# morrislab/rnascan

Measured on AMD Instinct MI355X. Metric: scored windows/sec (seq+struct, w=12), higher is better.
Workload: dtype f64

## Files before the change

### include/pfmscan.h

```cpp
#ifndef PFMSCAN_H
#define PFMSCAN_H

#include <stdint.h>

#ifdef __cplusplus
extern "C" {
#endif

#define PFMSCAN_ABI_VERSION 27
#define PFMSCAN_NCODE   8
#define PFMSCAN_SEP     7
#define PFMSCAN_NSTRUCT 7
#define PFMSCAN_MAX_M   64
#define PFMSCAN_MAX_WIDTH 4096
#define PFMSCAN_SITE_GROUP 4096
#define PFMSCAN_SITE_LIMBS 66
#define PFMSCAN_SITE_JOINT_COLS 64

#define PFMSCAN_OK          0
#define PFMSCAN_E_BADARG   -1
#define PFMSCAN_E_BADSHAPE -2
#define PFMSCAN_E_OOM      -3
#define PFMSCAN_E_HIP      -4
#define PFMSCAN_E_CAPACITY -5
// ... 151 lines not shown
int pfmscan_debug_pair_credits(const double *letters_seq, const double *letters_struct, int m, double thr_sum,
                               uint16_t *credits_seq, uint16_t *credits_struct, double *quantum, double *slack,
                               double *thr_joint, double *survive, int *mode);
int pfmscan_debug_pair_sum_test(const float *seq, const double *st, int64_t n, double thr_sum,
                                uint8_t *maybe, uint8_t *passes, double *margin0);

typedef struct pfmscan_library pfmscan_library;
int pfmscan_library_create(pfmscan_ctx *ctx, const double *letter_tables,
                           const double *struct_pssms, int n_motifs, int m,
                           pfmscan_library **out);
void pfmscan_library_destroy(pfmscan_library *lib);
int pfmscan_library_info(const pfmscan_library *lib, int *n_motifs, int *m, int *n_passes,
                         int *motifs_per_pass, double *max_eps);
int pfmscan_library_last_launches(const pfmscan_library *lib, int *n_launches, int *n_team_launches,
                                  int *max_teams);
int pfmscan_library_hits_dev(pfmscan_ctx *ctx, pfmscan_library *lib,
                             const uint8_t *d_codes, const void *d_profile,
                             int profile_dtype, int64_t n_pos, const double *thr_seq,
                             const double *thr_struct, int64_t capacity,
                             int64_t *d_hit_pos, int32_t *d_hit_motif, float *d_hit_seq,
                             double *d_hit_struct, uint64_t *d_hit_count, void *stream);
int pfmscan_library_hits_staged(pfmscan_ctx *ctx, pfmscan_library *lib,
                                const double *thr_seq, const double *thr_struct,
                                int64_t capacity, int64_t *hit_pos, int32_t *hit_motif,
                                float *hit_seq, double *hit_struct, int64_t *n_hits);
int pfmscan_library_hits_host(pfmscan_ctx *ctx, pfmscan_library *lib,
                              const uint8_t *codes, const void *profile, int profile_dtype,
                              int64_t n_pos, const double *thr_seq, const double *thr_struct,
                              int64_t capacity, int64_t *hit_pos, int32_t *hit_motif,
                              float *hit_seq, double *hit_struct, int64_t *n_hits);
// ... 48 lines not shown
                                         int64_t *d_hit_pos, int32_t *d_hit_motif, float *d_hit_seq,
                                         double *d_hit_struct, uint64_t *d_hit_count, void *stream);
int pfmscan_library_hits_letters_sum_host(pfmscan_ctx *ctx, pfmscan_library *lib, const uint8_t *codes,
                                          const uint8_t *codes2, int64_t n_pos, const double *thr_seq,
                                          const double *thr_struct, const double *thr_sum, int64_t capacity,
                                          int64_t *hit_pos, int32_t *hit_motif, float *hit_seq,
                                          double *hit_struct, int64_t *n_hits);
int pfmscan_library_letters_sum_thresholds(const double *letter_tables, const double *struct_tables, int n_motifs,
                                           int m, const double *thr_seq, const double *thr_sum, double *thr_eff);

int pfmscan_debug_credit_table(const double *letter_table, int m, double thr_seq, int bits,
                               uint16_t *credits, double *slack);

int pfmscan_debug_library8_credits(const double *letter_table, int m, double thr, uint16_t *credits, double *slack);

int pfmscan_debug_credit8_table(const double *letter_table, int m, double thr, uint16_t *credits, int *mode);

#define PFMSCAN_UPLOAD_RUNTIME 0
#define PFMSCAN_UPLOAD_STAGED  1
int pfmscan_set_upload_mode(pfmscan_ctx *ctx, int mode);
int pfmscan_upload_source_file(pfmscan_ctx *ctx, const void *base, size_t length, const char *path, int64_t file_offset);
int pfmscan_upload_source_file_checked(pfmscan_ctx *ctx, const void *base, size_t length, const char *path,
                                       int64_t file_offset, int64_t st_dev, int64_t st_ino, int64_t st_size);

int pfmscan_dotbracket_annotate_dev(pfmscan_ctx *ctx, const uint8_t *d_in, uint8_t *d_out, int64_t n_pos,
                                    const uint8_t *map, int64_t *d_counts, int64_t *first_bad, void *stream);
int pfmscan_dotbracket_stage(pfmscan_ctx *ctx, const uint8_t *codes, int64_t n_pos, int which, const uint8_t *map,
                             int64_t *counts, int64_t *first_bad);
int pfmscan_dotbracket_annotate_host(pfmscan_ctx *ctx, const uint8_t *in, uint8_t *out, int64_t n_pos,
                                     const uint8_t *map, int64_t *counts, int64_t *first_bad);
// ... 297 lines not shown
```

### rnascan_amd/_lib.py

```python
import ctypes
import importlib.util
import os
import sys

import numpy as np

HERE = os.path.dirname(os.path.abspath(__file__))
LIB_PATH = os.environ.get("PFMSCAN_LIB") or os.path.join(HERE, "libpfmscan.so")

OK = 0
E_BADARG, E_BADSHAPE, E_OOM, E_HIP, E_CAPACITY = -1, -2, -3, -4, -5
PROFILE_NONE, PROFILE_F32, PROFILE_F64 = 0, 1, 2
SEP = 7
NCODE = 8
NSTRUCT = 7
MAX_M = 64
MAX_WIDTH = 4096
ABI_VERSION = 27

SYMBOLS = [
    "pfmscan_abi_version", "pfmscan_ctx_create", "pfmscan_ctx_destroy", "pfmscan_last_error",
    "pfmscan_device_info", "pfmscan_synchronize", "pfmscan_motif_create", "pfmscan_motif_destroy",
    "pfmscan_pwm_calculate", "pfmscan_scan_dev", "pfmscan_scan_letters_f64_dev", "pfmscan_hits_dev",
    "pfmscan_scan_host", "pfmscan_scan_letters_f64_host", "pfmscan_hits_host", "pfmscan_time_scan_dev",
# ... 23 lines not shown
    "pfmscan_site_joint_dev", "pfmscan_site_joint_staged",
    "pfmscan_mutmap_dev", "pfmscan_mutmap_staged", "pfmscan_mutmap_events_dev", "pfmscan_mutmap_events_staged",
    "pfmscan_variants_dev", "pfmscan_variants_staged",
    "pfmscan_occupancy_dev", "pfmscan_occupancy_staged",
    "pfmscan_occupancy_profile_dev", "pfmscan_occupancy_profile_staged",
    "pfmscan_expect_dev", "pfmscan_expect_staged",
    "pfmscan_expect_profile_dev", "pfmscan_expect_profile_staged",
    "pfmscan_occupancy_pair_dev", "pfmscan_occupancy_pair_staged", "pfmscan_expect_pair_dev", "pfmscan_expect_pair_staged",
    "pfmscan_expect_merge_dev", "pfmscan_expect_merged_staged", "pfmscan_expect_profile_merged_staged", "pfmscan_expect_pair_merged_staged",
    "pfmscan_expect_pair_joint_dev", "pfmscan_expect_pair_joint_staged", "pfmscan_expect_pair_joint_merged_staged",
    "pfmscan_expect_profile_joint_dev", "pfmscan_expect_profile_joint_staged", "pfmscan_expect_profile_joint_merged_staged",
    "pfmscan_footprint_dev", "pfmscan_footprint_staged", "pfmscan_footprint_events_dev", "pfmscan_footprint_events_staged",
    "pfmscan_footprint_profile_dev", "pfmscan_footprint_profile_staged", "pfmscan_footprint_profile_events_dev", "pfmscan_footprint_profile_events_staged",
    "pfmscan_mutocc_dev", "pfmscan_mutocc_staged", "pfmscan_mutocc_events_dev", "pfmscan_mutocc_events_staged",
    "pfmscan_multisite_dev", "pfmscan_multisite_staged", "pfmscan_multisite_events_dev", "pfmscan_multisite_events_staged",
]
PAIR_ROUTE_NONE, PAIR_ROUTE_FUSED, PAIR_ROUTE_TWO_PHASE, PAIR_ROUTE_DENSE, PAIR_ROUTE_CREDITS = range(5)
SITE_GROUP = 4096
SITE_LIMBS = 66
SITE_JOINT_COLS = 64
EXPECT_RATIO, EXPECT_POSTERIOR = 0, 1
OCC_FANIN = 32
FOOTPRINT_SLOTS = 512
FOOTPRINT_PROFILE_SLOTS = 256
MULTISITE_SLOTS = 512
MULTISITE_CHUNK = 28
MUTOCC_TILE = 512
MAX_COVER = 1024
AVG_OK, AVG_DOTBRACKET, AVG_UNCOVERED, AVG_COVER, AVG_BAD_TABLE = range(5)
TSV_CONST, TSV_I64, TSV_F32, TSV_F64, TSV_INDEXED, TSV_FIXED, TSV_WINDOW, TSV_SPAN = range(8)

# ... 2045 lines not shown
                                                                 dtype=np.float64), (self.n,)))
        return ts, tt

    def info(self):
        n, m, npass, per, eps = ctypes.c_int(), ctypes.c_int(), ctypes.c_int(), ctypes.c_int(), ctypes.c_double()
        self._ctx._check(self._L.pfmscan_library_info(self._h, ctypes.byref(n), ctypes.byref(m), ctypes.byref(npass),
                                                      ctypes.byref(per), ctypes.byref(eps)))
        return {"n_motifs": n.value, "m": m.value, "passes": npass.value, "motifs_per_pass": per.value,
                "max_prefilter_eps": eps.value}

    def last_launches(self):
        n, teams, most = ctypes.c_int(), ctypes.c_int(), ctypes.c_int()
        self._ctx._check(self._L.pfmscan_library_last_launches(self._h, ctypes.byref(n), ctypes.byref(teams), ctypes.byref(most)))
        return {"n_launches": n.value, "n_team_launches": teams.value, "max_teams": most.value}

    def close(self):
        if getattr(self, "_h", None) and getattr(self._ctx, "_h", None):
            self._L.pfmscan_library_destroy(self._h)
        self._h = None

    def __del__(self):
        try:
            self.close()
        except Exception:
            pass


def credit_table(letter_table, thr_seq, bits=16):
    L = load()
    T = np.ascontiguousarray(letter_table, dtype=np.float64)
# ... 25 lines not shown


def library8_credits(letter_table, thr):
    L = load()
    T = np.ascontiguousarray(letter_table, dtype=np.float64)
    if T.ndim != 2 or T.shape[1] != NCODE:
        raise ValueError("letter_table must be [m][8]")
    rows = (T.shape[0] + 3) // 4 * 4
    out = np.zeros((rows, 8), dtype=np.uint16)
    slack = ctypes.c_double(0.0)
    L.pfmscan_debug_library8_credits.argtypes = [ctypes.c_void_p, ctypes.c_int, ctypes.c_double, ctypes.c_void_p, ctypes.POINTER(ctypes.c_double)]
    rc = L.pfmscan_debug_library8_credits(_ptr(T), T.shape[0], float(thr), _ptr(out), ctypes.byref(slack))
    if rc != OK:
        raise ValueError("pfmscan_debug_library8_credits: bad argument")
    return out, slack.value


def credit8_table(letter_table, thr):
    L = load()
    T = np.ascontiguousarray(letter_table, dtype=np.float64)
    if T.ndim != 2 or T.shape[1] != NCODE:
        raise ValueError("letter_table must be [m][8]")
    out = np.zeros((T.shape[0], 8), dtype=np.uint16)
    mode = ctypes.c_int(0)
    rc = L.pfmscan_debug_credit8_table(_ptr(T), T.shape[0], float(thr), _ptr(out), ctypes.byref(mode))
    if rc != OK:
        raise ValueError("pfmscan_debug_credit8_table: bad argument")
    return out, mode.value


# ... 26 lines not shown
```

### rnascan_amd/build.py

```python
import os
import re
import shutil
import subprocess
import sys
import tempfile
from concurrent.futures import ThreadPoolExecutor

HERE = os.path.dirname(os.path.abspath(__file__))
CSRC = os.path.join(HERE, "csrc")
OBJ = os.path.join(CSRC, "_obj")
LIB = os.path.join(HERE, "libpfmscan.so")
SOURCES = ["pfmscan_kernels.hip", "pfmscan_letters8.hip", "pfmscan_pairsum.hip", "pfmscan_letters_fixed.hip", "pfmscan_api.hip", "pfmscan_hits.hip", "pfmscan_sort.hip", "pfmscan_library.hip", "pfmscan_library_api.hip", "pfmscan_proflib.hip", "pfmscan_profile_fixed.hip", "pfmscan_place.hip",
           "pfmscan_pipeline.hip", "pfmscan_ingest.hip", "pfmscan_upload.hip", "pfmscan_dotbracket.hip", "pfmscan_average.hip", "pfmscan_background.hip", "pfmscan_rowbound.hip", "pfmscan_sites.hip", "pfmscan_sites_host.hip", "pfmscan_sites_lib.hip",
           "pfmscan_sites_lib_host.hip", "pfmscan_sites_letters.hip", "pfmscan_mutation.hip", "pfmscan_occupancy.hip", "pfmscan_expect.hip", "pfmscan_expect_profile.hip", "pfmscan_expect_merge.hip", "pfmscan_footprint.hip", "pfmscan_footprint_profile.hip", "pfmscan_mutocc.hip", "pfmscan_multisite.hip"]
HEADERS = ["pfmscan_internal.hpp", "pfmscan_ctx.hpp", "pfmscan_hits.hpp", "pfmscan_hitqueue.hpp", "pfmscan_device.hpp", "pfmscan_profile.hpp", "pfmscan_exact.hpp", "pfmscan_sites.hpp", "pfmscan_superacc.hpp", "pfmscan_occ.hpp", "pfmscan_occ_plan.hpp", "pfmscan_fp.hpp", "pfmscan_fp_plan.hpp", "pfmscan_ms_plan.hpp", os.path.join("..", "..", "include", "pfmscan.h")]
DEPS = SOURCES + HEADERS
FLAGS = ["-O3", "--offload-arch=gfx950", "-std=c++17", "-fPIC", "-fno-fast-math", "-Wall"]


def hipcc_path():
    for cand in (os.environ.get("HIPCC"), shutil.which("hipcc"), "/opt/rocm/bin/hipcc"):
        if cand and os.path.exists(cand):
            return cand
    raise RuntimeError("hipcc not found (set HIPCC or install ROCm under /opt/rocm)")


def stale():
    if not os.path.exists(LIB):
        return True
    t = os.path.getmtime(LIB)
# ... 78 lines not shown
```

### rnascan_amd/csrc/pfmscan_internal.hpp

```cpp
#pragma once
#include <hip/hip_runtime.h>
#include <stdint.h>
#include <atomic>
#include "../../include/pfmscan.h"

namespace pfmscan {

struct CredCache {
    double thr = __builtin_nan("");
    int mode = 0;
    uint16_t cr[16 * 16];
};

struct Cred8Cache {
    double thr = __builtin_nan("");
    int mode = 0;
    uint16_t cr[32 * 8];
};

struct PairCred {
    int mode = 0;
    int m = 0;
    double thr_sum = __builtin_nan("");
    double thr_joint = 0.0, quantum = 0.0, slack = 0.0, survive = 0.0;
// ... 166 lines not shown
    const double *thr;
    double struct_band;
    const int32_t *finite;
    int n_motifs, m, motif_base;
    int64_t pos_offset;
    int64_t capacity;
    int hit_shards;
    int64_t *hit_pos;
    int32_t *hit_motif;
    double *hit_struct;
    unsigned long long *hit_count;
};
hipError_t launch_profile_library(const ProfLibArgs &a, hipStream_t stream);
int64_t profile_library_tile();

hipError_t sort_temp_bytes(int64_t total, int key_bits, size_t *bytes);
hipError_t launch_gather_sorted(const GatherArgs &g, hipStream_t stream);

}
```

### rnascan_amd/csrc/pfmscan_library_api.hip

```cpp
#include <algorithm>
#include <cmath>
#include <cstdlib>
#include <cstring>
#include <new>
#include <string>
#include <vector>

#include "pfmscan_hits.hpp"

using namespace pfmscan;

namespace {

struct LibPass {
    int motif_base = 0, n_real = 0, nmp = 0, ng = 0;
    int ng_real = 0;
    size_t pairs_off = 0;
    size_t letters_off = 0;
    size_t pssm_off = 0;
    size_t thr_off = 0;
};

}

// ... 69 lines not shown
    bool all_finite = false;
    double struct_band = 0.0;
    std::vector<double> pairsum;
    std::vector<LibPass> passes;
    uint16_t *d_pairs = nullptr;
    double *d_letters = nullptr, *d_pssm = nullptr, *d_thr = nullptr;
    size_t pairs_elems = 0, thr_elems = 0;
    std::vector<uint16_t> h_pairs;
    std::vector<double> h_thr;
    std::vector<double> cur_seq, cur_struct, eps;
    std::vector<double> h_letters, h_pssm;
    std::vector<double> band;
    std::vector<double> cur_eff, cur_sum;
    bool thr_valid = false;
    int last_launches = 0, last_team_launches = 0, last_max_teams = 0;
};

static int lib_fail(pfmscan_ctx *ctx, int code, const std::string &msg) { return fail(ctx, code, msg); }

extern "C" {

static int create_seq_library(pfmscan_ctx *ctx, const double *letter_tables, const double *struct_pssms, int ncol, int n_motifs, int m,
                              pfmscan_library **out);

int pfmscan_library_create(pfmscan_ctx *ctx, const double *letter_tables, const double *struct_pssms, int n_motifs, int m,
                           pfmscan_library **out)
{
    if (!ctx || !out || (!letter_tables && !struct_pssms)) return lib_fail(ctx, PFMSCAN_E_BADARG, "pfmscan_library_create: NULL argument");
    *out = nullptr;
    if (n_motifs < 1 || n_motifs > 65535) return lib_fail(ctx, PFMSCAN_E_BADSHAPE, "library size outside 1..65535");
// ... 2 lines not shown
    if (!letter_tables) {
        HIP_TRY(ctx, hipSetDevice(ctx->device));
        pfmscan_library *lib = new (std::nothrow) pfmscan_library();
        if (!lib) return lib_fail(ctx, PFMSCAN_E_OOM, "out of host memory");
        lib->ctx = ctx;
        lib->n = n_motifs;
        lib->m = m;
        lib->has_struct = true;
        lib->has_letters = false;
        for (int k = 0; k < n_motifs; ++k) lib->struct_band = std::max(lib->struct_band, struct_band(struct_pssms + (size_t)k * m * 7, m));
        std::vector<int32_t> fin((size_t)n_motifs, 1);
        for (int k = 0; k < n_motifs; ++k)
            for (int i = 0; i < m * 7; ++i)
                if (!std::isfinite(struct_pssms[(size_t)k * m * 7 + i])) fin[(size_t)k] = 0;
        if (std::getenv("PFMSCAN_FORCE_GENERIC")) std::fill(fin.begin(), fin.end(), 0);
        const size_t cells = (size_t)n_motifs * m * 7;
        hipError_t e = hipMalloc((void **)&lib->d_pssm_rows, cells * 8);
        if (e == hipSuccess) e = hipMemcpy(lib->d_pssm_rows, struct_pssms, cells * 8, hipMemcpyHostToDevice);
        if (e == hipSuccess) e = hipMalloc((void **)&lib->d_finite, (size_t)n_motifs * 4);
        if (e == hipSuccess) e = hipMemcpy(lib->d_finite, fin.data(), (size_t)n_motifs * 4, hipMemcpyHostToDevice);
        if (e == hipSuccess) e = hipMalloc((void **)&lib->d_thr, (size_t)n_motifs * 8);
        lib->thr_elems = (size_t)n_motifs;
        if (e != hipSuccess) {
            pfmscan_library_destroy(lib);
            return fail_hip(ctx, e, "uploading the library tables");
        }
        *out = lib;
        return PFMSCAN_OK;
    }
    return create_seq_library(ctx, letter_tables, struct_pssms, 7, n_motifs, m, out);
}

}

static int create_seq_library(pfmscan_ctx *ctx, const double *letter_tables, const double *struct_pssms, int ncol, int n_motifs, int m,
                              pfmscan_library **out)
{
// ... 171 lines not shown
            return lib_fail(ctx, PFMSCAN_E_BADSHAPE, "column 7 of every letter table must be NaN (the foreign code)");
    if (seq_tables) return create_seq_library(ctx, seq_tables, struct_tables, 8, n_motifs, m, out);
    return create_letters8_library(ctx, struct_tables, n_motifs, m, out);
}

void pfmscan_library_destroy(pfmscan_library *lib)
{
    if (!lib) return;
    if (lib->ctx) (void)hipSetDevice(lib->ctx->device);
    if (lib->d_pairs) (void)hipFree(lib->d_pairs);
    if (lib->d_letters) (void)hipFree(lib->d_letters);
    if (lib->d_pssm) (void)hipFree(lib->d_pssm);
    if (lib->d_thr) (void)hipFree(lib->d_thr);
    if (lib->d_pssm_rows) (void)hipFree(lib->d_pssm_rows);
    if (lib->d_finite) (void)hipFree(lib->d_finite);
    delete lib;
}

int pfmscan_debug_credit_table(const double *letter_table, int m, double thr_seq, int bits, uint16_t *credits, double *slack)
{
    if (!letter_table || !credits || m < 1 || m > PFMSCAN_MAX_M || std::isnan(thr_seq)) return PFMSCAN_E_BADARG;
    if (bits == 0) bits = lib_credit_bits(lib_np_bucket(m));
    if (bits != 10 && bits != 16) return PFMSCAN_E_BADARG;
    const int npair = (m + 1) / 2;
    std::vector<double> ps((size_t)npair * 16);
    pair_sums(letter_table, m, ps.data());
    const double s = build_credits(ps.data(), npair, thr_seq, credits, bits);
    if (slack) *slack = s;
    return PFMSCAN_OK;
}
// ... 23 lines not shown
        for (double v : lib->eps) mx = std::max(mx, v);
        *max_eps = lib->thr_valid ? mx : NAN;
    }
    return PFMSCAN_OK;
}

int pfmscan_library_last_launches(const pfmscan_library *lib, int *n_launches, int *n_team_launches, int *max_teams)
{
    if (!lib) return PFMSCAN_E_BADARG;
    if (n_launches) *n_launches = lib->last_launches;
    if (n_team_launches) *n_team_launches = lib->last_team_launches;
    if (max_teams) *max_teams = lib->last_max_teams;
    return PFMSCAN_OK;
}

}

static int lib_set_thresholds(pfmscan_ctx *ctx, pfmscan_library *lib, const double *thr_seq, const double *thr_struct, hipStream_t st,
                              const double *thr_sum = nullptr, double row_sum_max = INFINITY)
{
    const int n = lib->n, npair = lib->npair;
    if (!lib->has_letters && !lib->letters8) {
        for (int k = 0; k < n; ++k)
            if (std::isnan(thr_struct[k])) return lib_fail(ctx, PFMSCAN_E_BADARG, "NaN threshold");
        if (lib->thr_valid && std::equal(thr_struct, thr_struct + n, lib->cur_struct.begin())) return PFMSCAN_OK;
        HIP_TRY(ctx, hipStreamSynchronize(st));
        lib->h_thr.assign(thr_struct, thr_struct + n);
        HIP_TRY(ctx, hipMemcpyAsync(lib->d_thr, lib->h_thr.data(), (size_t)n * 8, hipMemcpyHostToDevice, st));
        lib->cur_struct.assign(thr_struct, thr_struct + n);
        lib->eps.assign((size_t)n, 0.0);
        lib->thr_valid = true;
        return PFMSCAN_OK;
    }
    if (lib->letters8) {
        const int rows = lib->npair;
        for (int k = 0; k < n; ++k) {
            if (std::isnan(thr_struct[k])) return lib_fail(ctx, PFMSCAN_E_BADARG, "NaN threshold");
            if (thr_struct[k] == -INFINITY)
                return lib_fail(ctx, PFMSCAN_E_BADARG, "library hits need a finite threshold (every window would be a hit; use the all-scores entry points)");
        }
        if (lib->thr_valid && std::equal(thr_struct, thr_struct + n, lib->cur_struct.begin())) return PFMSCAN_OK;
        HIP_TRY(ctx, hipStreamSynchronize(st));
        lib->thr_valid = false;
// ... 127 lines not shown
                a.pos_offset = pos_offset;
                a.capacity = sink.shard_cap;
                a.hit_shards = sink.shards;
                a.hit_pos = sink.pos;
                a.hit_motif = sink.motif;
                a.hit_seq = nullptr;
                a.hit_struct = sink.st;
                a.hit_count = sink.count;
                hipError_t e = launch_library8(a, ctx->n_cu, st);
                if (e != hipSuccess) return fail_hip(ctx, e, "launch k_library8");
                lib_note_launch(lib, 1);
            }
        return PFMSCAN_OK;
    }
    if (!lib->has_letters) {
        ProfLibArgs a;
        std::memset(&a, 0, sizeof(a));
        a.profile = d_profile;
        a.profile_dtype = profile_dtype;
        a.n_pos = n_pos;
        a.pssm = lib->d_pssm_rows;
        a.thr = lib->d_thr;
        a.struct_band = lib->struct_band;
        a.finite = lib->d_finite;
        a.n_motifs = lib->n;
        a.m = lib->m;
        a.motif_base = 0;
        a.pos_offset = pos_offset;
        a.capacity = sink.shard_cap;
        a.hit_shards = sink.shards;
        a.hit_pos = sink.pos;
        a.hit_motif = sink.motif;
        a.hit_struct = sink.st;
        a.hit_count = sink.count;
        hipError_t e = launch_profile_library(a, st);
        if (e != hipSuccess) return fail_hip(ctx, e, "launch k_profile_lib");
        lib_note_launch(lib, 1);
        return PFMSCAN_OK;
    }
    const LibPass &first_pass = lib->passes[0];
    bool teams = lib->has_struct && !lib->pair && lib->passes.size() > 1 && n_pos >= (int64_t)8 * ctx->n_cu * LIB_SEG &&
                 ctx->n_cu >= 16 && !std::getenv("PFMSCAN_LIB_SEQUENTIAL");
    for (const LibPass &ps : lib->passes) teams = teams && ps.ng == first_pass.ng;
    const int64_t max_span = (int64_t)1 << 31;
    for (int64_t base = 0; base < n_pos; base += max_span) {
        const int64_t span_segs = (std::min<int64_t>(max_span, n_pos - base) + LIB_SEG - 1) / LIB_SEG;
        const size_t per_launch = teams && span_segs >= ctx->n_cu ? 4 : 1;
        for (size_t p0 = 0; p0 < lib->passes.size(); p0 += per_launch) {
            const LibPass &ps = lib->passes[p0];
            const size_t nt = std::min(per_launch, lib->passes.size() - p0);
            LibArgs a;
            std::memset(&a, 0, sizeof(a));
// ... 75 lines not shown
    if (lib->pair) {
        if (n_pos > 0 && !profile) return lib_fail(ctx, PFMSCAN_E_BADARG, "two-FASTA library: the second code stream is NULL");
        return PFMSCAN_OK;
    }
    if (lib->has_struct) {
        if (profile_dtype != PFMSCAN_PROFILE_F32 && profile_dtype != PFMSCAN_PROFILE_F64)
            return lib_fail(ctx, PFMSCAN_E_BADARG, "library has structure PSSMs: profile_dtype must be F32 or F64");
        if (n_pos > 0 && !profile) return lib_fail(ctx, PFMSCAN_E_BADARG, "library has structure PSSMs but profile is NULL");
    }
    return PFMSCAN_OK;
}

static int lib_acquire(pfmscan_ctx *ctx, pfmscan_library *lib, int64_t capacity, int64_t n_pos, hipStream_t st, HitSink &sink)
{
    lib->last_launches = lib->last_team_launches = lib->last_max_teams = 0;
    return acquire_sink(ctx, lib_bufs(ctx), LIB_SHARDS, lib_shard_cap(capacity, n_pos, lib_work_unit(lib)), st, sink);
}

namespace pfmscan {

constexpr int PACK_BLOCK = 256;

__global__ __launch_bounds__(PACK_BLOCK) void k_lib_prefix(const unsigned long long *__restrict__ counts, int shards,
                                                           int64_t shard_cap, int64_t capacity, int64_t *__restrict__ starts,
                                                           unsigned long long *__restrict__ out_count)
{
    __shared__ int64_t held[LIB_SHARDS];
    __shared__ unsigned long long total_s, worst_s;
    __shared__ int over_s;
    if (threadIdx.x == 0) {
// ... 314 lines not shown
```

Before: 150.9 billion.

## Add fp16 MFMA screening pass with exact f64 rescoring for profile libraries

Adds a new kernel that scores profile (structure-only) library motifs with f16 MFMA matrix products against a conservative per-motif cut derived from a rounding-error slack bound. Windows that may pass are queued and rescored exactly in f64, so most windows skip the expensive f64 dot products. Motifs with non-finite or too-large entries, or widths above 18, fall back to the existing exact kernel. This adds host-side planning, extra device tables and a survivor-batching path, and relies on the slack bound being truly conservative for correctness.

```diff
diff --git a/include/pfmscan.h b/include/pfmscan.h
--- a/include/pfmscan.h
+++ b/include/pfmscan.h
@@ -189,6 +189,8 @@
                          int *motifs_per_pass, double *max_eps);
 int pfmscan_library_last_launches(const pfmscan_library *lib, int *n_launches, int *n_team_launches,
                                   int *max_teams);
+int pfmscan_library_last_route(const pfmscan_library *lib, int *route, int *n_screened, int *n_exact, int64_t *survivors);
+void pfmscan_proflib_screen_info(int *tile, int *min_run, int *max_m, double *s_max);
 int pfmscan_library_hits_dev(pfmscan_ctx *ctx, pfmscan_library *lib,
                              const uint8_t *d_codes, const void *d_profile,
                              int profile_dtype, int64_t n_pos, const double *thr_seq,
@@ -267,6 +269,9 @@
 
 int pfmscan_debug_library8_credits(const double *letter_table, int m, double thr, uint16_t *credits, double *slack);
 
+int pfmscan_debug_proflib_screen(const double *struct_pssms, int n_motifs, int m, const double *thr, uint16_t *bhat,
+                                 double *slack, float *cut, int32_t *screened);
+
 int pfmscan_debug_credit8_table(const double *letter_table, int m, double thr, uint16_t *credits, int *mode);
 
 #define PFMSCAN_UPLOAD_RUNTIME 0
diff --git a/rnascan_amd/_lib.py b/rnascan_amd/_lib.py
--- a/rnascan_amd/_lib.py
+++ b/rnascan_amd/_lib.py
@@ -61,7 +61,9 @@
     "pfmscan_footprint_profile_dev", "pfmscan_footprint_profile_staged", "pfmscan_footprint_profile_events_dev", "pfmscan_footprint_profile_events_staged",
     "pfmscan_mutocc_dev", "pfmscan_mutocc_staged", "pfmscan_mutocc_events_dev", "pfmscan_mutocc_events_staged",
     "pfmscan_multisite_dev", "pfmscan_multisite_staged", "pfmscan_multisite_events_dev", "pfmscan_multisite_events_staged",
+    "pfmscan_library_last_route", "pfmscan_proflib_screen_info", "pfmscan_debug_proflib_screen",
 ]
+PROFLIB_ROUTE_NONE, PROFLIB_ROUTE_EXACT, PROFLIB_ROUTE_SCREEN, PROFLIB_ROUTE_MIXED = range(4)
 PAIR_ROUTE_NONE, PAIR_ROUTE_FUSED, PAIR_ROUTE_TWO_PHASE, PAIR_ROUTE_DENSE, PAIR_ROUTE_CREDITS = range(5)
 SITE_GROUP = 4096
 SITE_LIMBS = 66
@@ -2137,6 +2139,12 @@
         self._ctx._check(self._L.pfmscan_library_last_launches(self._h, ctypes.byref(n), ctypes.byref(teams), ctypes.byref(most)))
         return {"n_launches": n.value, "n_team_launches": teams.value, "max_teams": most.value}
 
+    def last_route(self):
+        route, ns, ne, sv = ctypes.c_int(), ctypes.c_int(), ctypes.c_int(), ctypes.c_int64()
+        self._L.pfmscan_library_last_route.argtypes = [ctypes.c_void_p] + [ctypes.POINTER(ctypes.c_int)] * 3 + [ctypes.POINTER(ctypes.c_int64)]
+        self._ctx._check(self._L.pfmscan_library_last_route(self._h, ctypes.byref(route), ctypes.byref(ns), ctypes.byref(ne), ctypes.byref(sv)))
+        return {"route": route.value, "n_screened": ns.value, "n_exact": ne.value, "survivors": sv.value}
+
     def close(self):
         if getattr(self, "_h", None) and getattr(self._ctx, "_h", None):
             self._L.pfmscan_library_destroy(self._h)
@@ -2192,6 +2200,31 @@
     if rc != OK:
         raise ValueError("pfmscan_debug_library8_credits: bad argument")
     return out, slack.value
+
+
+def proflib_screen_info():
+    L = load()
+    tile, run, mm, smax = ctypes.c_int(), ctypes.c_int(), ctypes.c_int(), ctypes.c_double()
+    L.pfmscan_proflib_screen_info.restype = None
+    L.pfmscan_proflib_screen_info.argtypes = [ctypes.POINTER(ctypes.c_int)] * 3 + [ctypes.POINTER(ctypes.c_double)]
+    L.pfmscan_proflib_screen_info(ctypes.byref(tile), ctypes.byref(run), ctypes.byref(mm), ctypes.byref(smax))
+    return {"tile": tile.value, "min_run": run.value, "max_m": mm.value, "s_max": smax.value}
+
+
+def proflib_screen_tables(struct_pssms, thr):
+    L = load()
+    P = np.ascontiguousarray(struct_pssms, dtype=np.float64)
+    if P.ndim != 3 or P.shape[2] != NSTRUCT:
+        raise ValueError("struct_pssms must be [n][m][7]")
+    n, m = P.shape[:2]
+    t = np.ascontiguousarray(np.broadcast_to(np.asarray(thr, dtype=np.float64), (n,)))
+    bhat = np.zeros((n, 2 * ((m + 1) // 2), 8), dtype=np.uint16)
+    slack, cut, scr = np.zeros(n, dtype=np.float64), np.zeros(n, dtype=np.float32), np.zeros(n, dtype=np.int32)
+    L.pfmscan_debug_proflib_screen.argtypes = [ctypes.c_void_p, ctypes.c_int, ctypes.c_int] + [ctypes.c_void_p] * 5
+    rc = L.pfmscan_debug_proflib_screen(_ptr(P), n, m, _ptr(t), _ptr(bhat), _ptr(slack), _ptr(cut), _ptr(scr))
+    if rc != OK:
+        raise ValueError("pfmscan_debug_proflib_screen: bad argument (NaN threshold, or a width outside 1..18)")
+    return bhat.view(np.float16), slack, cut, scr.astype(bool)
 
 
 def credit8_table(letter_table, thr):
diff --git a/rnascan_amd/build.py b/rnascan_amd/build.py
--- a/rnascan_amd/build.py
+++ b/rnascan_amd/build.py
@@ -10,10 +10,10 @@
 CSRC = os.path.join(HERE, "csrc")
 OBJ = os.path.join(CSRC, "_obj")
 LIB = os.path.join(HERE, "libpfmscan.so")
-SOURCES = ["pfmscan_kernels.hip", "pfmscan_letters8.hip", "pfmscan_pairsum.hip", "pfmscan_letters_fixed.hip", "pfmscan_api.hip", "pfmscan_hits.hip", "pfmscan_sort.hip", "pfmscan_library.hip", "pfmscan_library_api.hip", "pfmscan_proflib.hip", "pfmscan_profile_fixed.hip", "pfmscan_place.hip",
+SOURCES = ["pfmscan_kernels.hip", "pfmscan_letters8.hip", "pfmscan_pairsum.hip", "pfmscan_letters_fixed.hip", "pfmscan_api.hip", "pfmscan_hits.hip", "pfmscan_sort.hip", "pfmscan_library.hip", "pfmscan_library_api.hip", "pfmscan_proflib.hip", "pfmscan_proflib_screen.hip", "pfmscan_profile_fixed.hip", "pfmscan_place.hip",
            "pfmscan_pipeline.hip", "pfmscan_ingest.hip", "pfmscan_upload.hip", "pfmscan_dotbracket.hip", "pfmscan_average.hip", "pfmscan_background.hip", "pfmscan_rowbound.hip", "pfmscan_sites.hip", "pfmscan_sites_host.hip", "pfmscan_sites_lib.hip",
            "pfmscan_sites_lib_host.hip", "pfmscan_sites_letters.hip", "pfmscan_mutation.hip", "pfmscan_occupancy.hip", "pfmscan_expect.hip", "pfmscan_expect_profile.hip", "pfmscan_expect_merge.hip", "pfmscan_footprint.hip", "pfmscan_footprint_profile.hip", "pfmscan_mutocc.hip", "pfmscan_multisite.hip"]
-HEADERS = ["pfmscan_internal.hpp", "pfmscan_ctx.hpp", "pfmscan_hits.hpp", "pfmscan_hitqueue.hpp", "pfmscan_device.hpp", "pfmscan_profile.hpp", "pfmscan_exact.hpp", "pfmscan_sites.hpp", "pfmscan_superacc.hpp", "pfmscan_occ.hpp", "pfmscan_occ_plan.hpp", "pfmscan_fp.hpp", "pfmscan_fp_plan.hpp", "pfmscan_ms_plan.hpp", os.path.join("..", "..", "include", "pfmscan.h")]
+HEADERS = ["pfmscan_internal.hpp", "pfmscan_ctx.hpp", "pfmscan_hits.hpp", "pfmscan_hitqueue.hpp", "pfmscan_device.hpp", "pfmscan_profile.hpp", "pfmscan_exact.hpp", "pfmscan_sites.hpp", "pfmscan_superacc.hpp", "pfmscan_occ.hpp", "pfmscan_occ_plan.hpp", "pfmscan_fp.hpp", "pfmscan_fp_plan.hpp", "pfmscan_ms_plan.hpp", "pfmscan_proflib_screen.hpp", os.path.join("..", "..", "include", "pfmscan.h")]
 DEPS = SOURCES + HEADERS
 FLAGS = ["-O3", "--offload-arch=gfx950", "-std=c++17", "-fPIC", "-fno-fast-math", "-Wall"]
 
diff --git a/rnascan_amd/csrc/pfmscan_internal.hpp b/rnascan_amd/csrc/pfmscan_internal.hpp
--- a/rnascan_amd/csrc/pfmscan_internal.hpp
+++ b/rnascan_amd/csrc/pfmscan_internal.hpp
@@ -204,6 +204,33 @@
 hipError_t launch_profile_library(const ProfLibArgs &a, hipStream_t stream);
 int64_t profile_library_tile();
 
+struct ProfLibScreenArgs {
+    const void *profile;
+    int profile_dtype;
+    int64_t n_pos;
+    const double *pssm;
+    const double *thr;
+    double struct_band;
+    const uint16_t *bhat;
+    const float *cut;
+    const int32_t *ids;
+    int n_pad;
+    int m, motif_base;
+    int64_t pos_offset;
+    int64_t capacity;
+    int hit_shards;
+    int64_t *hit_pos;
+    int32_t *hit_motif;
+    double *hit_struct;
+    unsigned long long *hit_count;
+    unsigned long long *survivors;
+    int64_t n_tiles, shard_positions;
+    int tiles_per_wg;
+};
+hipError_t launch_profile_library_screen(const ProfLibScreenArgs &a, int n_cu, hipStream_t stream);
+int64_t profile_library_screen_tile();
+int64_t profile_library_screen_min_run();
+
 hipError_t sort_temp_bytes(int64_t total, int key_bits, size_t *bytes);
 hipError_t launch_gather_sorted(const GatherArgs &g, hipStream_t stream);
 
diff --git a/rnascan_amd/csrc/pfmscan_library_api.hip b/rnascan_amd/csrc/pfmscan_library_api.hip
--- a/rnascan_amd/csrc/pfmscan_library_api.hip
+++ b/rnascan_amd/csrc/pfmscan_library_api.hip
@@ -4,9 +4,11 @@
 #include <cstring>
 #include <new>
 #include <string>
+#include <utility>
 #include <vector>
 
 #include "pfmscan_hits.hpp"
+#include "pfmscan_proflib_screen.hpp"
 
 using namespace pfmscan;
 
@@ -107,6 +109,14 @@
     std::vector<double> cur_eff, cur_sum;
     bool thr_valid = false;
     int last_launches = 0, last_team_launches = 0, last_max_teams = 0;
+    std::vector<int32_t> h_finite;
+    ScreenPlan screen;
+    bool screen_ready = false;
+    uint16_t *d_bhat = nullptr;
+    float *d_cut = nullptr;
+    int32_t *d_ids = nullptr;
+    unsigned long long *d_survivors = nullptr;
+    int last_route = 0, last_screened = 0, last_exact = 0;
 };
 
 static int lib_fail(pfmscan_ctx *ctx, int code, const std::string &msg) { return fail(ctx, code, msg); }
@@ -139,6 +149,10 @@
             for (int i = 0; i < m * 7; ++i)
                 if (!std::isfinite(struct_pssms[(size_t)k * m * 7 + i])) fin[(size_t)k] = 0;
         if (std::getenv("PFMSCAN_FORCE_GENERIC")) std::fill(fin.begin(), fin.end(), 0);
+        lib->h_finite = fin;
+        lib->h_pssm.assign(struct_pssms, struct_pssms + (size_t)n_motifs * m * 7);
+        lib->band.resize((size_t)n_motifs);
+        for (int k = 0; k < n_motifs; ++k) lib->band[(size_t)k] = struct_band(struct_pssms + (size_t)k * m * 7, m);
         const size_t cells = (size_t)n_motifs * m * 7;
         hipError_t e = hipMalloc((void **)&lib->d_pssm_rows, cells * 8);
         if (e == hipSuccess) e = hipMemcpy(lib->d_pssm_rows, struct_pssms, cells * 8, hipMemcpyHostToDevice);
@@ -146,6 +160,14 @@
         if (e == hipSuccess) e = hipMemcpy(lib->d_finite, fin.data(), (size_t)n_motifs * 4, hipMemcpyHostToDevice);
         if (e == hipSuccess) e = hipMalloc((void **)&lib->d_thr, (size_t)n_motifs * 8);
         lib->thr_elems = (size_t)n_motifs;
+        if (m <= PLS_MAX_M) {
+            const size_t n_pad = ((size_t)n_motifs + PLS_SLAB - 1) / PLS_SLAB * PLS_SLAB;
+            if (e == hipSuccess) e = hipMalloc((void **)&lib->d_bhat, n_pad * (size_t)pls_ks(m) * 16 * 2);
+            if (e == hipSuccess) e = hipMalloc((void **)&lib->d_cut, n_pad * 4);
+            if (e == hipSuccess) e = hipMalloc((void **)&lib->d_ids, n_pad * 4);
+            if (e == hipSuccess) e = hipMalloc((void **)&lib->d_survivors, 8);
+            if (e == hipSuccess) e = hipMemset(lib->d_survivors, 0, 8);
+        }
         if (e != hipSuccess) {
             pfmscan_library_destroy(lib);
             return fail_hip(ctx, e, "uploading the library tables");
@@ -347,6 +369,10 @@
     if (lib->d_thr) (void)hipFree(lib->d_thr);
     if (lib->d_pssm_rows) (void)hipFree(lib->d_pssm_rows);
     if (lib->d_finite) (void)hipFree(lib->d_finite);
+    if (lib->d_bhat) (void)hipFree(lib->d_bhat);
+    if (lib->d_cut) (void)hipFree(lib->d_cut);
+    if (lib->d_ids) (void)hipFree(lib->d_ids);
+    if (lib->d_survivors) (void)hipFree(lib->d_survivors);
     delete lib;
 }
 
@@ -400,6 +426,65 @@
     return PFMSCAN_OK;
 }
 
+int pfmscan_library_last_route(const pfmscan_library *lib, int *route, int *n_screened, int *n_exact, int64_t *survivors)
+{
+    if (!lib) return PFMSCAN_E_BADARG;
+    if (route) *route = lib->last_route;
+    if (n_screened) *n_screened = lib->last_screened;
+    if (n_exact) *n_exact = lib->last_exact;
+    if (survivors) {
+        *survivors = 0;
+        if (lib->d_survivors && lib->last_route >= 2) {
+            unsigned long long v = 0;
+            if (lib->ctx) (void)hipSetDevice(lib->ctx->device);
+            if (hipDeviceSynchronize() != hipSuccess || hipMemcpy(&v, lib->d_survivors, 8, hipMemcpyDeviceToHost) != hipSuccess)
+                return PFMSCAN_E_HIP;
+            *survivors = (int64_t)v;
+        }
+    }
+    return PFMSCAN_OK;
+}
+
+void pfmscan_proflib_screen_info(int *tile, int *min_run, int *max_m, double *s_max)
+{
+    if (tile) *tile = (int)profile_library_screen_tile();
+    if (min_run) *min_run = (int)profile_library_screen_min_run();
+    if (max_m) *max_m = PLS_MAX_M;
+    if (s_max) *s_max = (double)PLS_SMAX;
+}
+
+int pfmscan_debug_proflib_screen(const double *struct_pssms, int n_motifs, int m, const double *thr, uint16_t *bhat, double *slack,
+                                 float *cut, int32_t *screened)
+{
+    if (!struct_pssms || !thr || !bhat || !slack || !cut || !screened || n_motifs < 1 || m < 1 || m > PLS_MAX_M) return PFMSCAN_E_BADARG;
+    std::vector<int32_t> fin((size_t)n_motifs, 1);
+    std::vector<double> band((size_t)n_motifs);
+    double lib_band = 0.0;
+    for (int k = 0; k < n_motifs; ++k) {
+        if (std::isnan(thr[k])) return PFMSCAN_E_BADARG;
+        for (int i = 0; i < m * 7; ++i)
+            if (!std::isfinite(struct_pssms[(size_t)k * m * 7 + i])) fin[(size_t)k] = 0;
+        band[(size_t)k] = struct_band(struct_pssms + (size_t)k * m * 7, m);
+        lib_band = std::max(lib_band, band[(size_t)k]);
+    }
+    const ScreenPlan sp = pls_plan(struct_pssms, n_motifs, m, thr, fin.data(), band.data(), lib_band);
+    const size_t per = (size_t)pls_ks(m) * 16;
+    std::memset(bhat, 0, (size_t)n_motifs * per * 2);
+    for (int k = 0; k < n_motifs; ++k) {
+        slack[k] = 0.0;
+        cut[k] = -INFINITY;
+        screened[k] = 0;
+    }
+    for (int i = 0; i < sp.n_screen; ++i) {
+        const int k = sp.ids[(size_t)i];
+        std::memcpy(bhat + (size_t)k * per, sp.bhat.data() + (size_t)i * per, per * 2);
+        slack[k] = sp.slack[(size_t)i];
+        cut[k] = sp.cut[(size_t)i];
+        screened[k] = 1;
+    }
+    return PFMSCAN_OK;
+}
+
 }
 
 static int lib_set_thresholds(pfmscan_ctx *ctx, pfmscan_library *lib, const double *thr_seq, const double *thr_struct, hipStream_t st,
@@ -413,6 +498,17 @@
         HIP_TRY(ctx, hipStreamSynchronize(st));
         lib->h_thr.assign(thr_struct, thr_struct + n);
         HIP_TRY(ctx, hipMemcpyAsync(lib->d_thr, lib->h_thr.data(), (size_t)n * 8, hipMemcpyHostToDevice, st));
+        lib->screen_ready = false;
+        if (lib->d_bhat) {
+            lib->screen = pls_plan(lib->h_pssm.data(), n, lib->m, thr_struct, lib->h_finite.data(), lib->band.data(), lib->struct_band);
+            const ScreenPlan &sp = lib->screen;
+            if (sp.n_pad > 0) {
+                HIP_TRY(ctx, hipMemcpyAsync(lib->d_bhat, sp.bhat.data(), sp.bhat.size() * 2, hipMemcpyHostToDevice, st));
+                HIP_TRY(ctx, hipMemcpyAsync(lib->d_cut, sp.cut.data(), sp.cut.size() * 4, hipMemcpyHostToDevice, st));
+                HIP_TRY(ctx, hipMemcpyAsync(lib->d_ids, sp.ids.data(), sp.ids.size() * 4, hipMemcpyHostToDevice, st));
+            }
+            lib->screen_ready = true;
+        }
         lib->cur_struct.assign(thr_struct, thr_struct + n);
         lib->eps.assign((size_t)n, 0.0);
         lib->thr_valid = true;
@@ -570,28 +666,71 @@
         return PFMSCAN_OK;
     }
     if (!lib->has_letters) {
-        ProfLibArgs a;
-        std::memset(&a, 0, sizeof(a));
-        a.profile = d_profile;
-        a.profile_dtype = profile_dtype;
-        a.n_pos = n_pos;
-        a.pssm = lib->d_pssm_rows;
-        a.thr = lib->d_thr;
-        a.struct_band = lib->struct_band;
-        a.finite = lib->d_finite;
-        a.n_motifs = lib->n;
-        a.m = lib->m;
-        a.motif_base = 0;
-        a.pos_offset = pos_offset;
-        a.capacity = sink.shard_cap;
-        a.hit_shards = sink.shards;
-        a.hit_pos = sink.pos;
-        a.hit_motif = sink.motif;
-        a.hit_struct = sink.st;
-        a.hit_count = sink.count;
-        hipError_t e = launch_profile_library(a, st);
-        if (e != hipSuccess) return fail_hip(ctx, e, "launch k_profile_lib");
-        lib_note_launch(lib, 1);
+        const char *sw = std::getenv("PFMSCAN_PROFLIB_SCREEN");
+        const bool screen = lib->screen_ready && lib->screen.n_screen > 0 && !(sw && sw[0] == '0' && sw[1] == 0);
+        std::vector<std::pair<int, int>> runs;
+        if (!screen)
+            runs.push_back({0, lib->n});
+        else
+            for (int32_t k : lib->screen.excluded) {
+                if (!runs.empty() && runs.back().second == k) ++runs.back().second;
+                else runs.push_back({k, k + 1});
+            }
+        if (screen) {
+            ProfLibScreenArgs s;
+            std::memset(&s, 0, sizeof(s));
+            s.profile = d_profile;
+            s.profile_dtype = profile_dtype;
+            s.n_pos = n_pos;
+            s.pssm = lib->d_pssm_rows;
+            s.thr = lib->d_thr;
+            s.struct_band = lib->struct_band;
+            s.bhat = lib->d_bhat;
+            s.cut = lib->d_cut;
+            s.ids = lib->d_ids;
+            s.n_pad = lib->screen.n_pad;
+            s.m = lib->m;
+            s.motif_base = 0;
+            s.pos_offset = pos_offset;
+            s.capacity = sink.shard_cap;
+            s.hit_shards = sink.shards;
+            s.hit_pos = sink.pos;
+            s.hit_motif = sink.motif;
+            s.hit_struct = sink.st;
+            s.hit_count = sink.count;
+            s.survivors = lib->d_survivors;
+            hipError_t e = launch_profile_library_screen(s, ctx->n_cu, st);
+            if (e != hipSuccess) return fail_hip(ctx, e, "launch k_profile_lib_screen");
+            lib_note_launch(lib, 1);
+            lib->last_screened = lib->screen.n_screen;
+        }
+        lib->last_exact = 0;
+        for (const std::pair<int, int> &r : runs) lib->last_exact += r.second - r.first;
+        lib->last_route = screen ? (runs.empty() ? 2 : 3) : 1;
+        for (const std::pair<int, int> &r : runs) {
+            ProfLibArgs a;
+            std::memset(&a, 0, sizeof(a));
+            a.profile = d_profile;
+            a.profile_dtype = profile_dtype;
+            a.n_pos = n_pos;
+            a.pssm = lib->d_pssm_rows + (size_t)r.first * lib->m * 7;
+            a.thr = lib->d_thr + r.first;
+            a.struct_band = lib->struct_band;
+            a.finite = lib->d_finite + r.first;
+            a.n_motifs = r.second - r.first;
+            a.m = lib->m;
+            a.motif_base = r.first;
+            a.pos_offset = pos_offset;
+            a.capacity = sink.shard_cap;
+            a.hit_shards = sink.shards;
+            a.hit_pos = sink.pos;
+            a.hit_motif = sink.motif;
+            a.hit_struct = sink.st;
+            a.hit_count = sink.count;
+            hipError_t e = launch_profile_library(a, st);
+            if (e != hipSuccess) return fail_hip(ctx, e, "launch k_profile_lib");
+            lib_note_launch(lib, 1);
+        }
         return PFMSCAN_OK;
     }
     const LibPass &first_pass = lib->passes[0];
@@ -697,6 +836,11 @@
 static int lib_acquire(pfmscan_ctx *ctx, pfmscan_library *lib, int64_t capacity, int64_t n_pos, hipStream_t st, HitSink &sink)
 {
     lib->last_launches = lib->last_team_launches = lib->last_max_teams = 0;
+    lib->last_route = lib->last_screened = lib->last_exact = 0;
+    if (lib->d_survivors) {
+        hipError_t e = hipMemsetAsync(lib->d_survivors, 0, 8, st);
+        if (e != hipSuccess) return fail_hip(ctx, e, "zeroing the survivor counter");
+    }
     return acquire_sink(ctx, lib_bufs(ctx), LIB_SHARDS, lib_shard_cap(capacity, n_pos, lib_work_unit(lib)), st, sink);
 }
 
diff --git a/rnascan_amd/csrc/pfmscan_proflib_screen.hip b/rnascan_amd/csrc/pfmscan_proflib_screen.hip
--- /dev/null
+++ b/rnascan_amd/csrc/pfmscan_proflib_screen.hip
@@ -0,0 +1,284 @@
+#include <float.h>
+#include <math.h>
+
+#include "pfmscan_internal.hpp"
+#include "pfmscan_exact.hpp"
+#include "pfmscan_hitqueue.hpp"
+#include "pfmscan_proflib_screen.hpp"
+
+namespace pfmscan {
+
+constexpr int PS_BLOCK = 256;
+constexpr int PS_WAVES = PS_BLOCK / 64;
+constexpr int PS_TILE = 256;
+constexpr int PS_SVCAP = 128;
+constexpr int PS_MIN_RUN = 4;
+
+typedef _Float16 ps_h8 __attribute__((ext_vector_type(8)));
+typedef float ps_f16 __attribute__((ext_vector_type(16)));
+
+int64_t profile_library_screen_tile() { return PS_TILE; }
+int64_t profile_library_screen_min_run() { return PS_MIN_RUN; }
+
+template <typename PROF_T> struct PsRow { PROF_T x[7]; };
+
+template <typename PROF_T>
+__device__ __forceinline__ void ps_load_row(const PROF_T *__restrict__ profile, int64_t pos, int64_t n_pos, PsRow<PROF_T> &r)
+{
+    if (pos < n_pos) {
+        const PROF_T *src = profile + pos * 7;
+#pragma unroll
+        for (int c = 0; c < 7; ++c) r.x[c] = src[c];
+    } else {
+#pragma unroll
+        for (int c = 0; c < 7; ++c) r.x[c] = (PROF_T)0;
+    }
+}
+
+template <typename PROF_T>
+__device__ __forceinline__ bool ps_store_row(ps_h8 *image, int row, const PsRow<PROF_T> &r)
+{
+    float f[7], sum = 0.0f, lo = 0.0f;
+#pragma unroll
+    for (int c = 0; c < 7; ++c) {
+        f[c] = (float)r.x[c];
+        sum += fabsf(f[c]);
+        lo = fminf(lo, f[c]);
+    }
+    const bool ok = (sum <= PLS_SMAX) && (lo >= 0.0f);
+    ps_h8 h;
+#pragma unroll
+    for (int c = 0; c < 7; ++c) h[c] = (_Float16)f[c];
+    h[7] = (_Float16)0.0f;
+    image[row] = h;
+    return ok;
+}
+
+template <typename PROF_T>
+__device__ __forceinline__ double ps_window_fast(const PROF_T *__restrict__ rows, const double *__restrict__ pssm, int m)
+{
+    double acc = 0.0;
+#pragma unroll 1
+    for (int j = 0; j < m; ++j) {
+#pragma unroll
+        for (int k = 0; k < 7; ++k) acc = fma((double)rows[j * 7 + k], pssm[j * 7 + k], acc);
+    }
+    return acc;
+}
+
+template <typename PROF_T>
+__device__ __forceinline__ double ps_window_slow(const PROF_T *__restrict__ rows, const double *__restrict__ pssm, int m)
+{
+    double score = 0.0;
+#pragma unroll 1
+    for (int j = 0; j < m; ++j) {
+        double d = (double)rows[j * 7] * pssm[j * 7];
+#pragma unroll 1
+        for (int k = 1; k < 7; ++k) d = fma((double)rows[j * 7 + k], pssm[j * 7 + k], d);
+        score += exact_nan_to_num(d);
+    }
+    return score;
+}
+
+template <typename PROF_T, int KS>
+__global__ __launch_bounds__(PS_BLOCK) void k_profile_lib_screen(const ProfLibScreenArgs a)
+{
+    constexpr int HALO = 2 * KS;
+    __shared__ __align__(16) ps_h8 s_image[2][PS_TILE + HALO];
+    __shared__ unsigned long long s_sv[PS_WAVES][PS_SVCAP];
+    __shared__ uint32_t s_flag[2];
+
+    const int tid = threadIdx.x;
+    const int lane = tid & 63;
+    const int wave = __builtin_amdgcn_readfirstlane(tid >> 6);
+    const int m = a.m;
+    const int64_t n_pos = a.n_pos;
+    const PROF_T *__restrict__ profile = reinterpret_cast<const PROF_T *>(a.profile);
+
+    const int64_t tile_first = (int64_t)blockIdx.x * a.tiles_per_wg;
+    const int64_t tiles_left = a.n_tiles - tile_first;
+    const int n_run = (int)(tiles_left < a.tiles_per_wg ? tiles_left : (int64_t)a.tiles_per_wg);
+    const int64_t pos_first = tile_first * PS_TILE;
+
+    if (tid < 2) s_flag[tid] = 0u;
+
+    unsigned long long *sv = s_sv[wave];
+    int sv_n = 0;
+    uint32_t n_surv = 0;
+
+    auto exact_batch = [&](int at, int cnt) {
+        __builtin_amdgcn_fence(__ATOMIC_RELEASE, "wavefront");
+        __builtin_amdgcn_wave_barrier();
+        __builtin_amdgcn_fence(__ATOMIC_ACQUIRE, "wavefront");
+        bool hit = false;
+        int64_t p = 0;
+        int32_t q = 0;
+        double score = 0.0;
+        if (lane < cnt) {
+            const unsigned long long e = sv[at + lane];
+            p = pos_first + (int64_t)(e >> 20);
+            q = a.ids[(uint32_t)(e & 0xFFFFFu)];
+            const PROF_T *rows = profile + p * 7;
+            const double *pssm = a.pssm + (size_t)q * m * 7;
+            const double t = a.thr[q];
+            score = ps_window_fast(rows, pssm, m);
+            if (!(fabs(score) <= DBL_MAX)) score = ps_window_slow(rows, pssm, m);
+            const double t_lo = t - a.struct_band, t_hi = t + a.struct_band;
+            hit = score > t_lo;
+            if (hit && score <= t_hi) {
+                score = struct_window_rounded(rows, m, [&](int j, int c) { return pssm[j * 7 + c]; });
+                hit = score > t;
+            }
+        }
+        n_surv += (uint32_t)cnt;
+        const uint32_t shard = (uint32_t)((p / a.shard_positions) & (int64_t)(a.hit_shards - 1));
+        unsigned long long left = __builtin_amdgcn_ballot_w64(hit);
+        while (left) {
+            const int leader = __builtin_ctzll(left);
+            const uint32_t s = (uint32_t)__builtin_amdgcn_readlane((int)shard, leader);
+            const bool mine = hit && shard == s;
+            const unsigned long long mk = __builtin_amdgcn_ballot_w64(mine);
+            unsigned long long base = 0;
+            if (lane == leader) base = atomicAdd(a.hit_count + (size_t)s * HIT_COUNTER_STRIDE, (unsigned long long)__popcll(mk));
+            const uint32_t lo = (uint32_t)__builtin_amdgcn_readlane((int)(uint32_t)base, leader);
+            const uint32_t hi = (uint32_t)__builtin_amdgcn_readlane((int)(uint32_t)(base >> 32), leader);
+            base = ((unsigned long long)hi << 32) | lo;
+            if (mine) {
+                const unsigned long long slot = base + __builtin_amdgcn_mbcnt_hi((uint32_t)(mk >> 32), __builtin_amdgcn_mbcnt_lo((uint32_t)mk, 0u));
+                if ((int64_t)slot < a.capacity) {
+                    const unsigned long long o = (unsigned long long)s * (unsigned long long)a.capacity + slot;
+                    a.hit_pos[o] = p + a.pos_offset;
+                    a.hit_motif[o] = a.motif_base + q;
+                    a.hit_struct[o] = score;
+                }
+            }
+            left &= ~mk;
+        }
+        __builtin_amdgcn_fence(__ATOMIC_RELEASE, "wavefront");
+        __builtin_amdgcn_wave_barrier();
+    };
+
+    uint32_t stamp = 0;
+#pragma unroll 1
+    for (int slab = 0; slab < a.n_pad; slab += PLS_SLAB) {
+        ps_h8 bfrag[2][KS];
+        float cut[2];
+        uint32_t midx[2];
+        bool valid[2];
+#pragma unroll
+        for (int cs = 0; cs < 2; ++cs) {
+            midx[cs] = (uint32_t)(slab + wave * 64 + cs * 32 + (lane & 31));
+            const _Float16 *b = reinterpret_cast<const _Float16 *>(a.bhat) + (size_t)midx[cs] * (KS * 16) + 8 * (lane >> 5);
+#pragma unroll
+            for (int s = 0; s < KS; ++s) bfrag[cs][s] = *reinterpret_cast<const ps_h8 *>(b + s * 16);
+            cut[cs] = a.cut[midx[cs]];
+            valid[cs] = a.ids[midx[cs]] >= 0;
+        }
+
+        PsRow<PROF_T> r0, r1;
+        ps_load_row(profile, pos_first + tid, n_pos, r0);
+        if (tid < HALO) ps_load_row(profile, pos_first + PS_TILE + tid, n_pos, r1);
+#pragma unroll 1
+        for (int t = 0; t < n_run; ++t) {
+            ++stamp;
+            const int buf = t & 1;
+            const int64_t tile0 = pos_first + (int64_t)t * PS_TILE;
+            bool ok = ps_store_row(s_image[buf], tid, r0);
+            if (tid < HALO) ok = ps_store_row(s_image[buf], PS_TILE + tid, r1) && ok;
+            if (!ok) s_flag[buf] = stamp;
+            if (t + 1 < n_run) {
+                ps_load_row(profile, tile0 + PS_TILE + tid, n_pos, r0);
+                if (tid < HALO) ps_load_row(profile, tile0 + 2 * PS_TILE + tid, n_pos, r1);
+            }
+            __syncthreads();
+            const bool flagged = s_flag[buf] == stamp;
+            const int64_t live_all = n_pos - m + 1 - tile0;
+            const int live_n = live_all < 0 ? 0 : (live_all > PS_TILE ? PS_TILE : (int)live_all);
+            const ps_h8 *image = s_image[buf];
+#pragma unroll 1
+            for (int blk = 0; blk < PS_TILE / 32; ++blk) {
+                ps_h8 afrag[KS];
+#pragma unroll
+                for (int s = 0; s < KS; ++s) afrag[s] = image[blk * 32 + (lane & 31) + 2 * s + (lane >> 5)];
+                ps_f16 acc[2];
+#pragma unroll
+                for (int cs = 0; cs < 2; ++cs) {
+#pragma unroll
+                    for (int i = 0; i < 16; ++i) acc[cs][i] = 0.0f;
+#pragma unroll
+                    for (int s = 0; s < KS; ++s) acc[cs] = __builtin_amdgcn_mfma_f32_32x32x16_f16(afrag[s], bfrag[cs][s], acc[cs], 0, 0, 0);
+                }
+#pragma unroll
+                for (int cs = 0; cs < 2; ++cs) {
+                    float mx = acc[cs][0];
+#pragma unroll
+                    for (int i = 1; i < 16; ++i) mx = fmaxf(mx, acc[cs][i]);
+                    const bool any = valid[cs] && (flagged || !(mx <= cut[cs]));
+                    if (__builtin_amdgcn_ballot_w64(any) == 0) continue;
+#pragma unroll
+                    for (int i = 0; i < 16; ++i) {
+                        const int win = blk * 32 + (i & 3) + 8 * (i >> 2) + 4 * (lane >> 5);
+                        const bool s = any && (flagged || !(acc[cs][i] <= cut[cs])) && win < live_n;
+                        const unsigned long long sb = __builtin_amdgcn_ballot_w64(s);
+                        if (sb == 0) continue;
+                        if (s) {
+                            const int slot = sv_n + (int)__builtin_amdgcn_mbcnt_hi((uint32_t)(sb >> 32), __builtin_amdgcn_mbcnt_lo((uint32_t)sb, 0u));
+                            sv[slot] = ((unsigned long long)(uint32_t)(t * PS_TILE + win) << 20) | (unsigned long long)midx[cs];
+                        }
+                        sv_n += __popcll(sb);
+                        if (sv_n >= 64) {
+                            exact_batch(sv_n - 64, 64);
+                            sv_n -= 64;
+                        }
+                    }
+                }
+            }
+        }
+        __syncthreads();
+    }
+    if (sv_n > 0) exact_batch(0, sv_n);
+    if (a.survivors && lane == 0 && n_surv) atomicAdd(a.survivors, (unsigned long long)n_surv);
+}
+
+template <typename PROF_T, int KS>
+static hipError_t ps_launch(const ProfLibScreenArgs &a, unsigned grid, hipStream_t stream)
+{
+    hipLaunchKernelGGL((k_profile_lib_screen<PROF_T, KS>), dim3(grid), dim3(PS_BLOCK), 0, stream, a);
+    return hipGetLastError();
+}
+
+template <typename PROF_T>
+static hipError_t ps_launch_ks(const ProfLibScreenArgs &a, unsigned grid, hipStream_t stream)
+{
+    switch (pls_ks(a.m)) {
+    case 1: return ps_launch<PROF_T, 1>(a, grid, stream);
+    case 2: return ps_launch<PROF_T, 2>(a, grid, stream);
+    case 3: return ps_launch<PROF_T, 3>(a, grid, stream);
+    case 4: return ps_launch<PROF_T, 4>(a, grid, stream);
+    case 5: return ps_launch<PROF_T, 5>(a, grid, stream);
+    case 6: return ps_launch<PROF_T, 6>(a, grid, stream);
+    case 7: return ps_launch<PROF_T, 7>(a, grid, stream);
+    case 8: return ps_launch<PROF_T, 8>(a, grid, stream);
+    case 9: return ps_launch<PROF_T, 9>(a, grid, stream);
+    }
+    return hipErrorInvalidValue;
+}
+
+hipError_t launch_profile_library_screen(const ProfLibScreenArgs &args, int n_cu, hipStream_t stream)
+{
+    if (args.n_pos <= 0 || args.n_pad <= 0) return hipSuccess;
+    if (args.m < 1 || args.m > PLS_MAX_M || args.n_pad % PLS_SLAB != 0 || args.n_pad > (1 << 20)) return hipErrorInvalidValue;
+    ProfLibScreenArgs a = args;
+    a.n_tiles = (a.n_pos + PS_TILE - 1) / PS_TILE;
+    const int64_t want = (int64_t)(n_cu > 0 ? n_cu : 256) * 32;
+    int64_t run = (a.n_tiles + want - 1) / want;
+    if (run < PS_MIN_RUN) run = PS_MIN_RUN;
+    if (run > 32768) run = 32768;
+    a.tiles_per_wg = (int)run;
+    const int64_t grid = (a.n_tiles + run - 1) / run;
+    if (grid > 0x7FFFFFFF) return hipErrorInvalidValue;
+    a.shard_positions = profile_library_tile();
+    return a.profile_dtype == PFMSCAN_PROFILE_F64 ? ps_launch_ks<double>(a, (unsigned)grid, stream) : ps_launch_ks<float>(a, (unsigned)grid, stream);
+}
+
+}
diff --git a/rnascan_amd/csrc/pfmscan_proflib_screen.hpp b/rnascan_amd/csrc/pfmscan_proflib_screen.hpp
--- /dev/null
+++ b/rnascan_amd/csrc/pfmscan_proflib_screen.hpp
@@ -0,0 +1,119 @@
+#pragma once
+#include <cmath>
+#include <cstdint>
+#include <cstring>
+#include <vector>
+
+namespace pfmscan {
+
+constexpr float PLS_SMAX = 1.0009765625f;
+constexpr double PLS_S = 1.0009765625 * (1.0 + 0x1p-19);
+constexpr double PLS_P_MAX = 65504.0;
+constexpr int PLS_MAX_M = 18;
+constexpr int PLS_SLAB = 256;
+
+inline int pls_ks(int m) { return (m + 1) / 2; }
+
+inline uint16_t pls_f16_bits(double v)
+{
+    const uint16_t sign = std::signbit(v) ? 0x8000u : 0u;
+    const double a = std::fabs(v);
+    if (a == 0.0) return sign;
+    int e;
+    (void)std::frexp(a, &e);
+    int exp = e - 1;
+    if (exp < -14) exp = -14;
+    const double q = std::ldexp(a, 10 - exp);
+    double r = std::nearbyint(q);
+    if (r >= 2048.0) {
+        r = 1024.0;
+        ++exp;
+    }
+    const uint32_t mant = (uint32_t)r;
+    if (mant < 1024u) return (uint16_t)(sign | mant);
+    return (uint16_t)(sign | (uint32_t)((exp + 15) << 10) | (mant - 1024u));
+}
+
+inline double pls_up(double x) { return std::nextafter(x, INFINITY); }
+inline double pls_down(double x) { return std::nextafter(x, -INFINITY); }
+
+inline bool pls_motif_ok(const double *pssm, int m, double thr)
+{
+    if (!std::isfinite(thr)) return false;
+    for (int i = 0; i < m * 7; ++i)
+        if (!(std::fabs(pssm[i]) <= PLS_P_MAX)) return false;
+    return true;
+}
+
+inline double pls_slack(const double *pssm, int m, double band)
+{
+    double F = 0.0, pmax = 0.0;
+    for (int j = 0; j < m; ++j) {
+        double mx = 0.0;
+        for (int c = 0; c < 7; ++c) mx = std::fmax(mx, std::fabs(pssm[j * 7 + c]));
+        F = pls_up(F + mx);
+        pmax = std::fmax(pmax, mx);
+    }
+    const double SF = pls_up(PLS_S * F);
+    const double quant = pls_up(SF * (0x1p-10 + 0x1p-21));
+    const double sub = pls_up(8.0 * (double)m * 0x1p-25 * pls_up(pmax + PLS_S));
+    const double acc = pls_up(2.0 * 16.0 * (double)pls_ks(m) * 0x1p-24 * pls_up(SF + sub));
+    return pls_up(pls_up(pls_up(quant + sub) + acc) + band);
+}
+
+inline float pls_cut(double thr, double lib_band, double slack)
+{
+    const double d = pls_down(pls_down(thr - lib_band) - slack);
+    float f = (float)d;
+    if ((double)f > d) f = std::nextafterf(f, -INFINITY);
+    return f;
+}
+
+inline void pls_operand(const double *pssm, int m, uint16_t *out)
+{
+    const int ks = pls_ks(m);
+    std::memset(out, 0, (size_t)ks * 16 * sizeof(uint16_t));
+    for (int j = 0; j < m; ++j)
+        for (int c = 0; c < 7; ++c) out[j * 8 + c] = pls_f16_bits(pssm[j * 7 + c]);
+}
+
+struct ScreenPlan {
+    std::vector<int32_t> ids;
+    std::vector<uint16_t> bhat;
+    std::vector<float> cut;
+    std::vector<double> slack;
+    std::vector<int32_t> excluded;
+    int n_screen = 0, n_pad = 0;
+};
+
+inline ScreenPlan pls_plan(const double *pssms, int n, int m, const double *thr, const int32_t *finite, const double *band, double lib_band)
+{
+    ScreenPlan p;
+    if (m < 1 || m > PLS_MAX_M) {
+        for (int k = 0; k < n; ++k) p.excluded.push_back(k);
+        return p;
+    }
+    for (int k = 0; k < n; ++k) {
+        if (finite[k] && pls_motif_ok(pssms + (size_t)k * m * 7, m, thr[k]))
+            p.ids.push_back(k);
+        else
+            p.excluded.push_back(k);
+    }
+    p.n_screen = (int)p.ids.size();
+    p.n_pad = (p.n_screen + PLS_SLAB - 1) / PLS_SLAB * PLS_SLAB;
+    p.ids.resize((size_t)p.n_pad, -1);
+    const size_t per = (size_t)pls_ks(m) * 16;
+    p.bhat.assign((size_t)p.n_pad * per, (uint16_t)0);
+    p.cut.assign((size_t)p.n_pad, INFINITY);
+    p.slack.assign((size_t)p.n_pad, 0.0);
+    for (int i = 0; i < p.n_screen; ++i) {
+        const int k = p.ids[(size_t)i];
+        const double *P = pssms + (size_t)k * m * 7;
+        pls_operand(P, m, p.bhat.data() + (size_t)i * per);
+        p.slack[(size_t)i] = pls_slack(P, m, band[k]);
+        p.cut[(size_t)i] = pls_cut(thr[k], lib_band, p.slack[(size_t)i]);
+    }
+    return p;
+}
+
+}
```

New measurement: 150.3 billion. Within noise of the previous version (-0.4%).
